# tirr-c/jxl-oxide

Hardware: NVIDIA H100
Metric: Megapixels/s decoded (8K VarDCT d1.0) (higher is better)
Workload: dtype f32

## Files before the change

### jxl_oxide_b200/csrc/kernels/hf_lanes.cuh

```cuda
#pragma once
#include "kernels.h"
#include "stream_common.cuh"
#ifndef __CUDACC__
#include <cstring>
#include <vector>

#include "../launch_tables.h"
#endif

#ifndef JXLB_LANE_TRIP
#define JXLB_LANE_TRIP(is_coefficient)
#endif
#ifndef JXLB_LANE_LZ77_COPIED
#define JXLB_LANE_LZ77_COPIED(n)
#endif

namespace jxlb {
namespace {

#define JXLB_TABLE_QUAL __device__ __constant__ const
namespace hftab {
#include "../host/jxl_tables.inc"
}
#undef JXLB_TABLE_QUAL

__device__ __constant__ const uint8_t kTInfo[27][5] = {
    {1, 1, 0, 0, 1},  {1, 1, 1, 1, 0},  {1, 1, 2, 1, 0},   {1, 1, 3, 1, 0},    {2, 2, 4, 2, 1},   {4, 4, 5, 3, 1},
    {1, 2, 6, 4, 1},  {2, 1, 6, 4, 0},  {1, 4, 7, 5, 1},   {4, 1, 7, 5, 0},    {2, 4, 8, 6, 1},   {4, 2, 8, 6, 0},
    {1, 1, 9, 1, 0},  {1, 1, 9, 1, 0},  {1, 1, 10, 1, 0},  {1, 1, 10, 1, 0},   {1, 1, 10, 1, 0},  {1, 1, 10, 1, 0},
    {8, 8, 11, 7, 1}, {4, 8, 12, 8, 1}, {8, 4, 12, 8, 0},  {16, 16, 13, 9, 1}, {8, 16, 14, 10, 1}, {16, 8, 14, 10, 0},
    {32, 32, 15, 11, 1}, {16, 32, 16, 12, 1}, {32, 16, 16, 12, 0},
};

#ifdef __CUDACC__
struct HfLds {
  using Addr = uint32_t;
  static __device__ __forceinline__ Addr addr(const void* p) { return uint32_t(__cvta_generic_to_shared(p)); }
  static __device__ __forceinline__ uint32_t u8(Addr a) {
    uint32_t v;
    asm("ld.shared.u8 %0, [%1];" : "=r"(v) : "r"(a));
    return v;
  }
  static __device__ __forceinline__ uint32_t u32(Addr a) {
    uint32_t v;
    asm("ld.shared.u32 %0, [%1];" : "=r"(v) : "r"(a));
    return v;
  }
  static __device__ __forceinline__ uint2 u64(Addr a) {
    uint2 v;
    asm("ld.shared.v2.u32 {%0, %1}, [%2];" : "=r"(v.x), "=r"(v.y) : "r"(a));
    return v;
  }
  static __device__ __forceinline__ void st8(Addr a, uint32_t v) { asm volatile("st.shared.u8 [%0], %1;" ::"r"(a), "r"(v)); }
};
#endif

struct HfBits {
  const uint32_t* base;
  uint32_t widx, stop_idx;
  uint64_t buf;
  uint32_t ahead;
  int nbits;
  __device__ __forceinline__ void init(const uint8_t* d, uint64_t bit_pos, uint64_t bit_limit) {
    base = reinterpret_cast<const uint32_t*>(d);
    const uint32_t w = uint32_t(bit_pos >> 5), skip = uint32_t(bit_pos & 31);
    stop_idx = uint32_t((bit_limit + 31) >> 5) + 2;
    buf = uint64_t(__ldg(base + w)) >> skip;
    nbits = 32 - int(skip);
    buf |= uint64_t(__ldg(base + w + 1)) << nbits;
    nbits += 32;
    ahead = __ldg(base + w + 2);
    widx = w + 3;
  }
  __device__ __forceinline__ void refill() {
    buf |= uint64_t(ahead) << nbits;
    nbits += 32;
    ahead = widx <= stop_idx ? __ldg(base + widx) : 0u;
    ++widx;
  }
  __device__ __forceinline__ void top_up() {
    if (nbits < 32) refill();
  }
  __device__ __forceinline__ uint32_t take(uint32_t n) {
    const uint32_t v = uint32_t(buf) & (n >= 32 ? 0xffffffffu : ((1u << n) - 1));
    buf >>= n;
    nbits -= int(n);
    return v;
  }
  __device__ __forceinline__ uint64_t pos() const { return uint64_t(widx - 1) * 32 - uint64_t(nbits); }
  __device__ __forceinline__ bool past_word(uint32_t k) const { return widx > k + (uint32_t(nbits) >> 5); }
};

template <class Mem>
struct HfTables {
  typename Mem::Addr cfg, ans;
  const uint64_t* ans_g;
  const uint32_t* prefix;
  const uint32_t* prefix_meta;
  uint32_t log_alphabet_size, log_bucket, use_prefix;
};

template <class Mem, bool ANS_SMEM, bool PREFIX = true, bool TRACK = false>
__device__ __forceinline__ uint32_t hf_read_value(const HfTables<Mem>& T, HfBits& br, uint32_t& ans_state, uint32_t cl,
                                                  uint32_t past_k = 0, bool* past = nullptr) {
  const uint32_t cfg = Mem::u32(T.cfg + cl * 4);
  uint32_t token;
  if (PREFIX && T.use_prefix) {
    const uint32_t off = __ldg(T.prefix_meta + cl * 2), root_bits = __ldg(T.prefix_meta + cl * 2 + 1);
    const uint32_t peeked = uint32_t(br.buf) & 0x7fffu;
    uint32_t e = __ldg(T.prefix + off + (peeked & ((1u << root_bits) - 1)));
    if (e & 0x80000000u) {
      const uint32_t sb = (e >> 16) & 0xff;
      e = __ldg(T.prefix + off + (1u << root_bits) + (e & 0xffff) + ((peeked >> root_bits) & ((1u << sb) - 1)));
    }
    br.take((e >> 16) & 0xff);
    token = e & 0xffff;
  } else {
    const uint32_t state = ans_state;
    const uint32_t idx = state & 0xfff;
    const uint32_t i = idx >> T.log_bucket;
    const uint32_t pos = idx & ((1u << T.log_bucket) - 1);
    uint2 b;
    if (ANS_SMEM) {
      b = Mem::u64(T.ans + (((cl << T.log_alphabet_size) + i) << 3));
    } else {
      const uint64_t g = __ldg(T.ans_g + ((size_t(cl) << T.log_alphabet_size) + i));
      b = make_uint2(uint32_t(g), uint32_t(g >> 32));
    }
    const bool map_to_alias = pos >= ((b.x >> 8) & 0xff);
    const uint32_t hi = map_to_alias ? b.y : 0u;
    const uint32_t offset = (hi & 0xffff) + pos;
    const uint32_t dist = (b.x >> 16) ^ (hi >> 16);
    token = map_to_alias ? (b.x & 0xff) : i;
    uint32_t next = (state >> 12) * dist + offset;
    if (next < (1u << 16)) {
      if (TRACK) *past |= br.past_word(past_k);
      next = (next << 16) | br.take(16);
    }
    ans_state = next;
  }
  const uint32_t split_exponent = cfg & 0xff;
  const uint32_t split = 1u << split_exponent;
  if (token < split) return token;
  const uint32_t msb = (cfg >> 8) & 0xff, lsb = (cfg >> 16) & 0xff;
  const uint32_t in_token = msb + lsb;
  const uint32_t n = (split_exponent - in_token + ((token - split) >> in_token)) & 31;
  if (TRACK) *past |= br.past_word(past_k);
  br.top_up();
  const uint32_t rest = br.take(n);
  const uint32_t low = token & ((1u << lsb) - 1);
  uint32_t t = (token >> lsb) & ((1u << msb) - 1);
  t |= 1u << msb;
  return uint32_t((((uint64_t(t) << n) | rest) << lsb) | low);
}

struct HfLaneSmem {
  uint32_t ctxlut, small, configs, bctx, cmap, cmap_stride, nz, ans, total;
};
__host__ __device__ inline HfLaneSmem hf_lane_layout(const DevHfParams& p, uint32_t nthreads) {
  HfLaneSmem L;
  uint32_t off = 0;
  auto take = [&](uint32_t bytes) {
    uint32_t o = off;
    off += (bytes + 15) & ~15u;
    return o;
  };
  L.ctxlut = take(128);
  L.small = take((27 + 39) * 4);
  L.configs = take(p.code.num_clusters * 4);
  L.bctx = take(p.block_ctx_map_size);
  L.cmap_stride = 495 * p.num_block_clusters;
  const uint32_t cmap_bytes = L.cmap_stride * p.num_hf_presets;
  L.cmap = cmap_bytes <= kLaneCmapSmemBytes ? take(cmap_bytes) : 0xffffffffu;
  L.nz = take(96 * nthreads);
  uint32_t ab = p.code.use_prefix ? 0 : (p.code.num_clusters << p.code.log_alphabet_size) * 8;
  L.ans = (!p.code.use_prefix && ab <= kHfAnsSmemBytes) ? take(ab) : 0xffffffffu;
  L.total = off;
  return L;
}
__host__ __device__ inline bool hf_lane_staged(const DevHfParams& p, const HfLaneSmem& L) {
  return !p.code.lz77_enabled && !p.code.use_prefix && L.ans != 0xffffffffu && L.cmap != 0xffffffffu;
}

template <class Mem>
struct HfLaneView {
  using Addr = typename Mem::Addr;
  Addr tinfo;
  Addr order_offset;
  Addr ctx;
  Addr bctx;
  Addr nz;
  uint32_t nz_stride;
  Addr cmap;
  HfTables<Mem> code;
  const uint8_t* cmap_ptr;
  CodeView cv;
  uint32_t cmap_stride;
};

__device__ __forceinline__ uint32_t hf_umin(uint32_t a, uint32_t b) { return a < b ? a : b; }
__device__ __forceinline__ uint32_t hf_pack_tinfo(uint32_t t) {
  const uint32_t blocks_log = 31u - uint32_t(__clz(int(uint32_t(kTInfo[t][0]) * kTInfo[t][1])));
  return uint32_t(kTInfo[t][0]) | blocks_log << 8 | uint32_t(kTInfo[t][3]) << 16 | uint32_t(kTInfo[t][4]) << 24;
}
struct HfTinfo {
  uint32_t w8, num_blocks_log, order_id, transpose;
};
__device__ __forceinline__ HfTinfo hf_unpack_tinfo(uint32_t ti) {
  return HfTinfo{ti & 0xff, (ti >> 8) & 0xff, (ti >> 16) & 0xff, ti >> 24};
}

constexpr uint32_t kHfNoBlock = 0xffffffffu;
template <bool SUB>
__device__ __forceinline__ uint32_t hf_block_ctx_cell(const DevFrame& f, const DevHfParams& p, uint32_t bx, uint32_t by) {
  const size_t gi = size_t(by) * f.bw + bx;
  const int32_t t = f.blk_type[gi];
  if (t < 0) return kHfNoBlock;
  const int32_t qf = f.blk_mul[gi];
  const int32_t* thr = p.lf_thresholds;
  uint32_t lf_idx = 0;
  if (p.has_lf_quant) {
    const int32_t* thr_base[3] = {thr, thr + p.num_lf_thr[0], thr + p.num_lf_thr[0] + p.num_lf_thr[1]};
    for (int kk = 0; kk < 3; ++kk) {
      const int cc = kk == 0 ? 0 : (kk == 1 ? 2 : 1);
      lf_idx *= p.num_lf_thr[cc] + 1;
      if (p.num_lf_thr[cc]) {
        const int32_t q = SUB ? f.lf_quant[cc][size_t(by >> f.vshift[cc]) * f.bw + (bx >> f.hshift[cc])] : f.lf_quant[cc][gi];
#pragma unroll 1
        for (uint32_t i = 0; i < p.num_lf_thr[cc]; ++i)
          if (q > thr_base[cc][i]) ++lf_idx;
      }
    }
  }
  uint32_t hf_idx = 0;
#pragma unroll 1
  for (uint32_t i = 0; i < p.num_qf_thr; ++i)
    if (qf > int32_t(p.qf_thresholds[i])) ++hf_idx;
  const uint32_t lf_idx_mul = (p.num_lf_thr[0] + 1) * (p.num_lf_thr[1] + 1) * (p.num_lf_thr[2] + 1);
  return uint32_t(t) | (hf_idx * lf_idx_mul + lf_idx) << 8;
}

struct HfGroupRect {
  uint32_t bx0, by0, width, height;
};
__device__ __forceinline__ HfGroupRect hf_group_rect(const DevFrame& f, const DevHfParams& p, uint32_t group_idx) {
  const uint32_t gb = p.group_dim_blocks;
  HfGroupRect r;
  r.bx0 = group_idx % p.groups_per_row * gb;
  r.by0 = group_idx / p.groups_per_row * gb;
  r.width = hf_umin(gb, f.bw - r.bx0);
  r.height = hf_umin(gb, f.bh - r.by0);
  return r;
}
__device__ __forceinline__ uint2 hf_block_rec(uint32_t info, uint32_t x, uint32_t y) { return make_uint2(info, x | y << 16); }
template <bool SUB>
__device__ __forceinline__ bool hf_block_record(const DevFrame& f, const DevHfParams& p, const HfGroupRect& r, uint32_t i,
                                                uint2& rec) {
  const uint32_t x = i % r.width, y = i / r.width;
  const uint32_t info = hf_block_ctx_cell<SUB>(f, p, r.bx0 + x, r.by0 + y);
  rec = hf_block_rec(info, x, y);
  return info != kHfNoBlock;
}

template <bool SUB, bool STAGED, bool LZ77, class Mem>
__device__ __forceinline__ void hf_lane_stream(const uint8_t* __restrict__ cs, const DevFrame& f, const DevHfParams& p,
                                               const HfLaneView<Mem>& T, const uint2* __restrict__ list, uint32_t count,
                                               const DevHfJob& job, int first_pass, Lz77State* lz, uint64_t* end_bit,
                                               int* status) {
  static_assert(!(LZ77 && STAGED), "LZ77 codes run the general variant");
  using Addr = typename Mem::Addr;
  DevBitReader br;
  HfBits hb;
  int err = kDevOk;
  uint32_t hfp_bits = 0;
  while ((1u << hfp_bits) < p.num_hf_presets) ++hfp_bits;
  uint32_t hfp, ans_state;
  const uint32_t last_word = uint32_t((job.bit_limit + 31) >> 5);
  const uint32_t* stop_word = nullptr;
  bool past = false;
  if (STAGED) {
    hb.init(cs, job.bit_pos, job.bit_limit);
    hfp = hb.take(hfp_bits);
    hb.top_up();
    ans_state = hb.take(32);
    past = (job.bit_pos >> 5) > last_word + 1 || job.bit_pos + hfp_bits > uint64_t(last_word + 2) * 32;
  } else {
    br.init(cs, job.bit_pos, job.bit_limit);
    hfp = br.read(hfp_bits);
    ans_state = p.code.use_prefix ? 0x130000u : br.read(32);
    stop_word = br.origin + last_word + 4;
  }
  if (hfp >= p.num_hf_presets) {
    err = kDevInvalid;
    hfp = 0;
  }
  const uint32_t nbc = p.num_block_clusters;
  const Addr a_cmap = T.cmap + T.cmap_stride * hfp;
  const uint8_t* cluster_map = STAGED ? nullptr : T.cmap_ptr + size_t(T.cmap_stride) * hfp;
  const uint32_t lf_idx_mul = (p.num_lf_thr[0] + 1) * (p.num_lf_thr[1] + 1) * (p.num_lf_thr[2] + 1);
  const uint32_t hf_idx_mul = p.num_qf_thr + 1;

  const HfGroupRect r = hf_group_rect(f, p, job.group_idx);
  const uint32_t bx0 = r.bx0, by0 = r.by0;
  for (uint32_t i = 0; i < 96; ++i) Mem::st8(T.nz + i * T.nz_stride, 0);

  uint32_t x = 0, y = 0;
  uint32_t ci = 3;
  uint32_t w8 = 1, num_blocks = 1, num_blocks_log = 0, order_id = 0, transpose = 0, blk_ctx_idx = 0;
  uint32_t left = count;
  uint2 next = count ? __ldg(list) : make_uint2(0, 0);
  ++list;
  bool in_coeffs = false;
  uint32_t k = 0, size = 0, non_zeros = 0, prev_nonzero = 0, nzc_ctx = 0, block_ctx = 0;
  int c = 0;
  uint32_t sx = 0;
  Addr a_blk = a_cmap;
  const uint8_t* cmap = cluster_map;
  const uint32_t* order = p.orders;
  uint32_t* dst_base = f.coeff[0];

  while (err == kDevOk) {
    uint32_t cl;
    if (!in_coeffs) {
      bool found = false;
      while (!found) {
        if (ci >= 3) {
          if (left == 0) break;
          const uint2 rec = next;
          if (--left) next = __ldg(list++);
          x = rec.y & 0xffff;
          y = rec.y >> 16;
          const HfTinfo ti = hf_unpack_tinfo(Mem::u32(T.tinfo + (rec.x & 0xff) * 4));
          w8 = ti.w8;
          num_blocks_log = ti.num_blocks_log;
          num_blocks = 1u << num_blocks_log;
          order_id = ti.order_id;
          transpose = ti.transpose;
          blk_ctx_idx = rec.x >> 8;
          ci = 0;
        }
        const uint32_t slot = ci++;
        c = slot == 0 ? 1 : (slot == 1 ? 0 : 2);
        sx = x;
        uint32_t sy = y, sbx0 = bx0, sby0 = by0;
        if (SUB) {
          const uint32_t hs = f.hshift[c], vs = f.vshift[c];
          sx = x >> hs, sy = y >> vs, sbx0 = bx0 >> hs, sby0 = by0 >> vs;
          if (hs | vs) {
            if ((sx << hs) != x || (sy << vs) != y) continue;
            if (f.blk_type[size_t(by0 + sy) * f.bw + bx0 + sx] < 0) continue;
            if (num_blocks != 1) {
              err = kDevUnsupported;
              break;
            }
          }
        }
        const uint32_t idx = ((slot * 13 + order_id) * hf_idx_mul) * lf_idx_mul + blk_ctx_idx;
        block_ctx = Mem::u8(T.bctx + idx);
        const uint32_t nz_here = Mem::u8(T.nz + (uint32_t(c) * 32 + sx) * T.nz_stride);
        const uint32_t nz_left = sx ? Mem::u8(T.nz + (uint32_t(c) * 32 + sx - 1) * T.nz_stride) : 0;
        uint32_t predicted;
        if (sy == 0) predicted = sx == 0 ? 32 : nz_left;
        else if (sx == 0) predicted = nz_here;
        else predicted = (nz_here + nz_left + 1) >> 1;
        const uint32_t pidx = predicted >= 8 ? 4 + predicted / 2 : predicted;
        cl = STAGED ? Mem::u8(a_cmap + block_ctx + pidx * nbc) : cluster_map[block_ctx + pidx * nbc];
        dst_base = f.coeff[c] + (size_t(sby0 + sy) * 8) * f.cw + size_t(sbx0 + sx) * 8;
        found = true;
      }
      if (!found) break;
    } else {
      const uint32_t cctx = (nzc_ctx + Mem::u8(T.ctx + ((k - num_blocks) >> num_blocks_log))) * 2 + prev_nonzero;
      if (cctx >= 458) {
        err = kDevInvalid;
        break;
      }
      cl = STAGED ? Mem::u8(a_blk + cctx) : cmap[cctx];
    }

    JXLB_LANE_TRIP(in_coeffs);
    uint32_t value;
    if (STAGED) {
      hb.top_up();
      value = hf_read_value<Mem, true, false, true>(T.code, hb, ans_state, cl, last_word + 3, &past);
    } else {
      if constexpr (LZ77) {
        value = lz77_read_value(T.cv, p.code, *lz, ans_state, br, cl, 0, err);
        if (err != kDevOk) break;
      } else {
        value = cv_read_uint(br, Mem::u32(T.code.cfg + cl * 4), cv_read_symbol(T.cv, ans_state, br, cl));
      }
      past = br.next_word > stop_word;
    }
    if (past) {
      err = kDevOverrun;
      break;
    }

    if (!in_coeffs) {
      if (value > (63u << num_blocks_log)) {
        err = kDevInvalid;
        break;
      }
      const uint32_t nz_val = (value + num_blocks - 1) >> num_blocks_log;
      for (uint32_t dx = 0; dx < w8; ++dx) Mem::st8(T.nz + (uint32_t(c) * 32 + sx + dx) * T.nz_stride, nz_val);
      if (value == 0) continue;
      non_zeros = value;
      prev_nonzero = (non_zeros <= num_blocks * 4) ? 1 : 0;
      order = p.orders + Mem::u32(T.order_offset + (order_id * 3 + c) * 4);
      size = num_blocks * 64;
      if (STAGED) a_blk = a_cmap + block_ctx * 458 + 37 * nbc;
      else cmap = cluster_map + block_ctx * 458 + 37 * nbc;
      nzc_ctx = Mem::u8(T.ctx + 64 + ((non_zeros - 1) >> num_blocks_log));
      k = num_blocks;
      in_coeffs = k < size;
    } else {
      bool channel_done = false;
      if (value == 0) {
        prev_nonzero = 0;
      } else {
        const uint32_t o = __ldg(order + k);
        const uint32_t cvv = uint32_t(dev_unpack_signed(value)) << p.coeff_shift;
        uint32_t dx = o & 0xffff, dy = o >> 16;
        if (transpose) {
          const uint32_t tmp = dx;
          dx = dy;
          dy = tmp;
        }
        uint32_t* dst = dst_base + size_t(dy) * f.cw + dx;
        if (first_pass) *dst = cvv;
        else *dst += cvv;
        prev_nonzero = 1;
        if (--non_zeros == 0) channel_done = true;
        else nzc_ctx = Mem::u8(T.ctx + 64 + ((non_zeros - 1) >> num_blocks_log));
      }
      if (!channel_done && ++k >= size) channel_done = true;
      if (channel_done) {
        in_coeffs = false;
        if ((STAGED ? hb.pos() : br.pos()) > job.bit_limit) err = kDevOverrun;
      }
    }
  }
  const uint64_t end = STAGED ? hb.pos() : br.pos();
  if (err == kDevOk && !p.code.use_prefix && ans_state != 0x130000u) err = kDevBadStream;
  if (err == kDevOk && end > job.bit_limit) err = kDevOverrun;
  *end_bit = end;
  *status = err;
}

#ifndef __CUDACC__
struct HfHostMem {
  using Addr = uintptr_t;
  static Addr addr(const void* p) { return reinterpret_cast<uintptr_t>(p); }
  static uint32_t u8(Addr a) { return *reinterpret_cast<const uint8_t*>(a); }
  static uint32_t u32(Addr a) {
    uint32_t v;
    std::memcpy(&v, reinterpret_cast<const void*>(a), 4);
    return v;
  }
  static uint2 u64(Addr a) {
    uint2 v;
    std::memcpy(&v, reinterpret_cast<const void*>(a), 8);
    return v;
  }
  static void st8(Addr a, uint32_t v) { *reinterpret_cast<uint8_t*>(a) = uint8_t(v); }
};

struct HfLaneTables {
  const uint32_t* tinfo;
  const uint32_t* order_offset;
  const uint8_t* ctx;
  const uint32_t* cfg;
  const uint8_t* bctx;
  const uint8_t* cmap;
  uint32_t cmap_stride;
  CodeView cv;
};

template <bool SUB>
inline void hf_lane_decode(const uint8_t* cs, const DevFrame& f, const DevHfParams& p, const HfLaneTables& T,
                           const uint32_t* blk_ctx, const DevHfJob& job, uint8_t* nz, uint32_t nz_stride, int first_pass,
                           uint64_t* end_bit, int* status) {
  if (p.code.lz77_enabled && f.subsampled) {
    *end_bit = job.bit_pos;
    *status = kDevUnsupported;
    return;
  }
  const HfGroupRect r = hf_group_rect(f, p, job.group_idx);
  std::vector<uint2> list;
  for (uint32_t y = 0; y < r.height; ++y)
    for (uint32_t x = 0; x < r.width; ++x) {
      const uint32_t info = blk_ctx[size_t(r.by0 + y) * f.bw + r.bx0 + x];
      if (info != kHfNoBlock) list.push_back(hf_block_rec(info, x, y));
    }
  HfLaneView<HfHostMem> V;
  V.tinfo = HfHostMem::addr(T.tinfo);
  V.order_offset = HfHostMem::addr(T.order_offset);
  V.ctx = HfHostMem::addr(T.ctx);
  V.bctx = HfHostMem::addr(T.bctx);
  V.nz = HfHostMem::addr(nz);
  V.nz_stride = nz_stride;
  V.cmap = HfHostMem::addr(T.cmap);
  V.cmap_ptr = T.cmap;
  V.cmap_stride = T.cmap_stride;
  V.code.cfg = HfHostMem::addr(T.cfg);
  V.code.ans = HfHostMem::addr(T.cv.ans);
  V.code.ans_g = T.cv.ans;
  V.code.prefix = T.cv.prefix;
  V.code.prefix_meta = T.cv.prefix_meta;
  V.code.log_alphabet_size = T.cv.log_alphabet_size;
  V.code.log_bucket = 12 - T.cv.log_alphabet_size;
  V.code.use_prefix = T.cv.use_prefix;
  V.cv = T.cv;
  const uint2* recs = list.data();
  const uint32_t n = uint32_t(list.size());
  if (p.code.lz77_enabled) {
    std::vector<uint32_t> window(hf_lz77_window_entries(p.group_dim_blocks * 8));
    Lz77State lz;
    lz77_init(lz, window.data(), window.size());
    hf_lane_stream<SUB, false, true>(cs, f, p, V, recs, n, job, first_pass, &lz, end_bit, status);
    JXLB_LANE_LZ77_COPIED(lz.copied);
  } else if (hf_lane_staged(p, hf_lane_layout(p, nz_stride)))
    hf_lane_stream<SUB, true, false>(cs, f, p, V, recs, n, job, first_pass, nullptr, end_bit, status);
  else
    hf_lane_stream<SUB, false, false>(cs, f, p, V, recs, n, job, first_pass, nullptr, end_bit, status);
}
#endif

}
}
```

### jxl_oxide_b200/csrc/kernels/entropy.cu

```cuda
#include "kernels.h"

#include "stream_common.cuh"
#include "hf_lanes.cuh"

namespace jxlb {

namespace {


struct HfSmem {
  uint32_t ctxlut, configs, bctx, cmap, cmap_stride, ans, total;
};
__host__ __device__ inline HfSmem hf_layout(const DevHfParams& p) {
  HfSmem L;
  uint32_t off = 0;
  auto take = [&](uint32_t bytes) {
    uint32_t o = off;
    off += (bytes + 15) & ~15u;
    return o;
  };
  L.ctxlut = take(128);
  L.configs = take(p.code.num_clusters * 4);
  L.bctx = take(p.block_ctx_map_size);
  L.cmap_stride = 495 * p.num_block_clusters;
  L.cmap = take(L.cmap_stride * p.num_hf_presets);
  uint32_t ab = p.code.use_prefix ? 0 : (p.code.num_clusters << p.code.log_alphabet_size) * 8;
  L.ans = (!p.code.use_prefix && ab <= kHfAnsSmemBytes) ? take(ab) : 0xffffffffu;
  L.total = off;
  return L;
}

template <bool SUB, int W, bool ANS_SMEM>
__global__ void __launch_bounds__(W * 32) decode_hf_warp_kernel(const uint8_t* __restrict__ cs, DevFrame f, DevHfParams p,
                                                                const DevHfJob* __restrict__ jobs,
                                                                uint64_t* __restrict__ end_bits, int* __restrict__ status,
                                                                int num_jobs, int first_pass) {
  extern __shared__ __align__(16) uint8_t smem[];
  __shared__ uint32_t s_nz[W][3][32];
  const HfSmem L = hf_layout(p);
  const uint32_t tid = threadIdx.x, nthreads = blockDim.x, lane = tid & 31, warp = tid >> 5;
  uint8_t* s_ctx = smem + L.ctxlut;
  for (uint32_t i = tid; i < 63; i += nthreads) {
    s_ctx[i] = hftab::kCoeffFreqContext[i];
    s_ctx[64 + i] = hftab::kCoeffNumNonzeroContext[i];
  }
  uint32_t* s_cfg = reinterpret_cast<uint32_t*>(smem + L.configs);
  for (uint32_t i = tid; i < p.code.num_clusters; i += nthreads) s_cfg[i] = __ldg(p.code.configs + i);
  uint8_t* s_bctx = smem + L.bctx;
  for (uint32_t i = tid; i < p.block_ctx_map_size; i += nthreads) s_bctx[i] = __ldg(p.block_ctx_map + i);
  {
    uint8_t* dst = smem + L.cmap;
    const uint32_t n = L.cmap_stride * p.num_hf_presets;
    for (uint32_t i = tid; i < n; i += nthreads) dst[i] = __ldg(p.code.cluster_map + i);
  }
  if (ANS_SMEM) {
    uint4* s_ans = reinterpret_cast<uint4*>(smem + L.ans);
    const uint32_t quads = (p.code.num_clusters << p.code.log_alphabet_size) / 2;
    const uint4* src = reinterpret_cast<const uint4*>(p.code.ans);
    for (uint32_t i = tid; i < quads; i += nthreads) s_ans[i] = __ldg(src + i);
  }
  __syncthreads();
  const int job_idx = blockIdx.x * W + int(warp);
  if (job_idx >= num_jobs || lane != 0) return;

  HfTables<HfLds> T;
  T.cfg = HfLds::addr(s_cfg);
  T.ans = ANS_SMEM ? HfLds::addr(smem + L.ans) : 0;
  T.ans_g = p.code.ans;
  T.prefix = p.code.prefix;
  T.prefix_meta = p.code.prefix_meta;
  T.log_alphabet_size = p.code.log_alphabet_size;
  T.log_bucket = 12 - p.code.log_alphabet_size;
  T.use_prefix = p.code.use_prefix;
  const uint32_t a_ctx = HfLds::addr(s_ctx), a_bctx = HfLds::addr(s_bctx);

  const DevHfJob job = jobs[job_idx];
  HfBits br;
  br.init(cs, job.bit_pos, job.bit_limit);
  int err = kDevOk;
  uint32_t hfp_bits = 0;
  while ((1u << hfp_bits) < p.num_hf_presets) ++hfp_bits;
  uint32_t hfp = br.take(hfp_bits);
  if (hfp >= p.num_hf_presets) {
    err = kDevInvalid;
    hfp = 0;
  }
  const uint32_t nbc = p.num_block_clusters;
  const uint32_t a_cmap = HfLds::addr(smem + L.cmap) + hfp * L.cmap_stride;
  const uint32_t lf_idx_mul = (p.num_lf_thr[0] + 1) * (p.num_lf_thr[1] + 1) * (p.num_lf_thr[2] + 1);
  const uint32_t hf_idx_mul = p.num_qf_thr + 1;
  br.top_up();
  uint32_t ans_state = p.code.use_prefix ? 0x130000u : br.take(32);

  const uint32_t gx = job.group_idx % p.groups_per_row, gy = job.group_idx / p.groups_per_row;
  const uint32_t gb = p.group_dim_blocks;
  const uint32_t bx0 = gx * gb, by0 = gy * gb;
  const uint32_t width = min(gb, f.bw - bx0), height = min(gb, f.bh - by0);
  uint32_t(*nz_row)[32] = s_nz[warp];
  for (int c = 0; c < 3; ++c)
    for (int i = 0; i < 32; ++i) nz_row[c][i] = 0;
  const int32_t* thr_base[3] = {p.lf_thresholds, p.lf_thresholds + p.num_lf_thr[0],
                                p.lf_thresholds + p.num_lf_thr[0] + p.num_lf_thr[1]};

  for (uint32_t y = 0; y < height && err == kDevOk; ++y)
    for (uint32_t x = 0; x < width && err == kDevOk; ++x) {
      const size_t gi = size_t(by0 + y) * f.bw + bx0 + x;
      const int32_t t = f.blk_type[gi];
      if (t < 0) continue;
      const int32_t qf = f.blk_mul[gi];
      const uint32_t w8 = kTInfo[t][0], h8 = kTInfo[t][1];
      const uint32_t order_id = kTInfo[t][3];
      const bool transpose = kTInfo[t][4] != 0;
      const uint32_t num_blocks = w8 * h8;
      const uint32_t num_blocks_log = 31u - uint32_t(__clz(int(num_blocks)));
      uint32_t lf_idx = 0;
      if (p.has_lf_quant) {
        const int cs3[3] = {0, 2, 1};
#pragma unroll
        for (int k = 0; k < 3; ++k) {
          const int c = cs3[k];
          lf_idx *= p.num_lf_thr[c] + 1;
          if (p.num_lf_thr[c]) {
            const int32_t q = SUB ? f.lf_quant[c][size_t((by0 + y) >> f.vshift[c]) * f.bw + ((bx0 + x) >> f.hshift[c])] : f.lf_quant[c][gi];
            for (uint32_t i = 0; i < p.num_lf_thr[c]; ++i)
              if (q > thr_base[c][i]) ++lf_idx;
          }
        }
      }
      uint32_t hf_idx = 0;
      for (uint32_t i = 0; i < p.num_qf_thr; ++i)
        if (qf > int32_t(p.qf_thresholds[i])) ++hf_idx;
#pragma unroll 1
      for (int ci = 0; ci < 3 && err == kDevOk; ++ci) {
        const uint32_t ch_idx = uint32_t(ci) * 13 + order_id;
        const int c = (ci == 0) ? 1 : (ci == 1 ? 0 : 2);
        uint32_t sx = x, sy = y, sbx0 = bx0, sby0 = by0;
        if (SUB) {
          const uint32_t hs = f.hshift[c], vs = f.vshift[c];
          sx = x >> hs, sy = y >> vs, sbx0 = bx0 >> hs, sby0 = by0 >> vs;
          if (hs | vs) {
            if ((sx << hs) != x || (sy << vs) != y) continue;
            if (f.blk_type[size_t(by0 + sy) * f.bw + bx0 + sx] < 0) continue;
            if (num_blocks != 1) {
              err = kDevUnsupported;
              break;
            }
          }
        }
        const uint32_t idx = (ch_idx * hf_idx_mul + hf_idx) * lf_idx_mul + lf_idx;
        const uint32_t block_ctx = HfLds::u8(a_bctx + idx);
        uint32_t predicted;
        const uint32_t nz_here = nz_row[c][sx];
        const uint32_t nz_left = sx ? nz_row[c][sx - 1] : 0;
        if (sy == 0) predicted = sx == 0 ? 32 : nz_left;
        else if (sx == 0) predicted = nz_here;
        else predicted = (nz_here + nz_left + 1) >> 1;
        const uint32_t pidx = predicted >= 8 ? 4 + predicted / 2 : predicted;
        br.top_up();
        uint32_t non_zeros = hf_read_value<HfLds, ANS_SMEM>(T, br, ans_state, HfLds::u8(a_cmap + block_ctx + pidx * nbc));
        if (non_zeros > (63u << num_blocks_log)) {
          err = kDevInvalid;
          break;
        }
        const uint32_t nz_val = (non_zeros + num_blocks - 1) >> num_blocks_log;
        for (uint32_t dx = 0; dx < w8; ++dx) nz_row[c][sx + dx] = nz_val;
        if (non_zeros == 0) continue;
        uint32_t prev_nonzero = (non_zeros <= num_blocks * 4) ? 1 : 0;
        const uint32_t* order = p.orders + p.order_offset[order_id * 3 + c];
        const uint32_t size = num_blocks * 64;
        const uint32_t a_blk = a_cmap + block_ctx * 458 + 37 * nbc;
        uint32_t* plane = f.coeff[c];
        const size_t base = (size_t(sby0 + sy) * 8) * f.cw + size_t(sbx0 + sx) * 8;
        uint32_t nzc2 = HfLds::u8(a_ctx + 64 + ((non_zeros - 1) >> num_blocks_log)) * 2;
        for (uint32_t k = num_blocks, i = 0; k < size; ++k, ++i) {
          const uint32_t cctx = nzc2 + HfLds::u8(a_ctx + (i >> num_blocks_log)) * 2 + prev_nonzero;
          if (cctx >= 458) {
            err = kDevInvalid;
            break;
          }
          br.top_up();
          const uint32_t ucoeff = hf_read_value<HfLds, ANS_SMEM>(T, br, ans_state, HfLds::u8(a_blk + cctx));
          if (ucoeff == 0) {
            prev_nonzero = 0;
            continue;
          }
          const uint32_t o = __ldg(order + k);
          const uint32_t cvv = uint32_t(dev_unpack_signed(ucoeff)) << p.coeff_shift;
          uint32_t dx = o & 0xffff, dy = o >> 16;
          if (transpose) {
            const uint32_t tmp = dx;
            dx = dy;
            dy = tmp;
          }
          uint32_t* dst = plane + base + size_t(dy) * f.cw + dx;
          if (first_pass) *dst = cvv;
          else *dst += cvv;
          prev_nonzero = 1;
          if (--non_zeros == 0) break;
          nzc2 = HfLds::u8(a_ctx + 64 + ((non_zeros - 1) >> num_blocks_log)) * 2;
        }
        if (br.pos() > job.bit_limit) err = kDevOverrun;
      }
    }
  if (err == kDevOk && !p.code.use_prefix && ans_state != 0x130000u) err = kDevBadStream;
  if (err == kDevOk && br.pos() > job.bit_limit) err = kDevOverrun;
  end_bits[job_idx] = br.pos();
  status[job_idx] = err;
}


template <bool SUB>
__global__ void __launch_bounds__(256) hf_block_list_kernel(DevFrame f, DevHfParams p, uint2* __restrict__ list,
                                                            uint32_t* __restrict__ counts) {
  __shared__ uint32_t s_warp[8];
  const uint32_t g = blockIdx.x, tid = threadIdx.x, lane = tid & 31, warp = tid >> 5;
  const HfGroupRect r = hf_group_rect(f, p, g);
  const uint32_t n = r.width * r.height;
  uint2* out = list + size_t(g) * p.group_dim_blocks * p.group_dim_blocks;
  uint32_t base = 0;
  for (uint32_t i0 = 0; i0 < n; i0 += 256) {
    uint2 rec;
    const bool has = i0 + tid < n && hf_block_record<SUB>(f, p, r, i0 + tid, rec);
    const uint32_t ballot = __ballot_sync(0xffffffffu, has);
    if (lane == 0) s_warp[warp] = __popc(ballot);
    __syncthreads();
    uint32_t before = base, total = 0;
    for (uint32_t w = 0; w < 8; ++w) {
      before += w < warp ? s_warp[w] : 0;
      total += s_warp[w];
    }
    if (has) out[before + __popc(ballot & ((1u << lane) - 1))] = rec;
    base += total;
    __syncthreads();
  }
  if (tid == 0) counts[g] = base;
}

template <bool SUB, bool STAGED, bool LZ77>
__global__ void __launch_bounds__(128) decode_hf_lanes_kernel(const uint8_t* __restrict__ cs, DevFrame f, DevHfParams p,
                                                              const uint2* __restrict__ list,
                                                              const uint32_t* __restrict__ counts,
                                                              const DevHfJob* __restrict__ jobs,
                                                              uint64_t* __restrict__ end_bits, int* __restrict__ status,
                                                              int num_jobs, int first_pass,
                                                              uint32_t* lz_windows, uint32_t lz_window_len) {
  extern __shared__ __align__(16) uint8_t smem[];
  const uint32_t tid = threadIdx.x, nthreads = blockDim.x;
  const HfLaneSmem L = hf_lane_layout(p, nthreads);
  uint8_t* s_ctx = smem + L.ctxlut;
  for (uint32_t i = tid; i < 63; i += nthreads) {
    s_ctx[i] = hftab::kCoeffFreqContext[i];
    s_ctx[64 + i] = hftab::kCoeffNumNonzeroContext[i];
  }
  uint32_t* s_cfg = reinterpret_cast<uint32_t*>(smem + L.configs);
  for (uint32_t i = tid; i < p.code.num_clusters; i += nthreads) s_cfg[i] = __ldg(p.code.configs + i);
  uint8_t* s_bctx = smem + L.bctx;
  for (uint32_t i = tid; i < p.block_ctx_map_size; i += nthreads) s_bctx[i] = __ldg(p.block_ctx_map + i);
  uint32_t* s_small = reinterpret_cast<uint32_t*>(smem + L.small);
  for (uint32_t i = tid; i < 27; i += nthreads) s_small[i] = hf_pack_tinfo(i);
  for (uint32_t i = tid; i < 39; i += nthreads) s_small[27 + i] = p.order_offset[i];
  HfLaneView<HfLds> T;
  T.tinfo = HfLds::addr(s_small);
  T.order_offset = HfLds::addr(s_small + 27);
  T.ctx = HfLds::addr(s_ctx);
  T.bctx = HfLds::addr(s_bctx);
  T.nz = HfLds::addr(smem + L.nz + tid);
  T.nz_stride = nthreads;
  T.cmap_stride = L.cmap_stride;
  T.cmap = 0;
  T.cmap_ptr = p.code.cluster_map;
  if (L.cmap != 0xffffffffu) {
    uint8_t* s_cmap = smem + L.cmap;
    const uint32_t n = L.cmap_stride * p.num_hf_presets;
    for (uint32_t i = tid; i < n; i += nthreads) s_cmap[i] = __ldg(p.code.cluster_map + i);
    T.cmap = HfLds::addr(s_cmap);
    T.cmap_ptr = s_cmap;
  }
  T.code.cfg = HfLds::addr(s_cfg);
  T.code.ans = 0;
  T.code.ans_g = p.code.ans;
  T.code.prefix = p.code.prefix;
  T.code.prefix_meta = p.code.prefix_meta;
  T.code.log_alphabet_size = p.code.log_alphabet_size;
  T.code.log_bucket = 12 - p.code.log_alphabet_size;
  T.code.use_prefix = p.code.use_prefix;
  T.cv.log_alphabet_size = p.code.log_alphabet_size;
  T.cv.use_prefix = p.code.use_prefix;
  T.cv.configs = s_cfg;
  T.cv.ans = p.code.ans;
  T.cv.prefix = p.code.prefix;
  T.cv.prefix_meta = p.code.prefix_meta;
  if (L.ans != 0xffffffffu) {
    uint4* s_ans = reinterpret_cast<uint4*>(smem + L.ans);
    const uint32_t quads = (p.code.num_clusters << p.code.log_alphabet_size) / 2;
    const uint4* src = reinterpret_cast<const uint4*>(p.code.ans);
    for (uint32_t i = tid; i < quads; i += nthreads) s_ans[i] = __ldg(src + i);
    T.code.ans = HfLds::addr(s_ans);
    T.cv.ans = reinterpret_cast<const uint64_t*>(s_ans);
  }
  __syncthreads();
  const int job_idx = blockIdx.x * int(nthreads) + int(tid);
  if (job_idx >= num_jobs) return;
  const DevHfJob job = jobs[job_idx];
  const uint32_t gb = p.group_dim_blocks;
  if constexpr (LZ77) {
    Lz77State lz;
    lz77_init(lz, lz_windows + size_t(job_idx) * lz_window_len, lz_window_len);
    hf_lane_stream<SUB, STAGED, true>(cs, f, p, T, list + size_t(job.group_idx) * gb * gb, __ldg(counts + job.group_idx),
                                      job, first_pass, &lz, end_bits + job_idx, status + job_idx);
  } else {
    hf_lane_stream<SUB, STAGED, false>(cs, f, p, T, list + size_t(job.group_idx) * gb * gb, __ldg(counts + job.group_idx),
                                       job, first_pass, nullptr, end_bits + job_idx, status + job_idx);
  }
}

}

size_t hf_block_list_count(DevFrame f, DevHfParams p) {
  const uint32_t gb = p.group_dim_blocks;
  return size_t((f.bh + gb - 1) / gb) * p.groups_per_row;
}

void launch_hf_block_list(DevFrame f, DevHfParams p, uint2* list, uint32_t* counts, cudaStream_t stream) {
  const uint32_t groups = uint32_t(hf_block_list_count(f, p));
  if (f.subsampled) hf_block_list_kernel<true><<<groups, 256, 0, stream>>>(f, p, list, counts);
  else hf_block_list_kernel<false><<<groups, 256, 0, stream>>>(f, p, list, counts);
}

void launch_decode_hf_lanes(const uint8_t* cs, DevFrame f, DevHfParams p, const uint2* list, const uint32_t* counts,
                            const DevHfJob* jobs, uint64_t* end_bits, int* status, int num_jobs, int first_pass,
                            int streams_per_cta, cudaStream_t stream, uint32_t* lz_windows, uint32_t lz_window_len) {
  if (num_jobs <= 0) return;
  static const bool attr_set = [] {
    cudaFuncSetAttribute(decode_hf_lanes_kernel<false, false, false>, cudaFuncAttributeMaxDynamicSharedMemorySize, 200 * 1024);
    cudaFuncSetAttribute(decode_hf_lanes_kernel<true, false, false>, cudaFuncAttributeMaxDynamicSharedMemorySize, 200 * 1024);
    cudaFuncSetAttribute(decode_hf_lanes_kernel<false, true, false>, cudaFuncAttributeMaxDynamicSharedMemorySize, 200 * 1024);
    cudaFuncSetAttribute(decode_hf_lanes_kernel<true, true, false>, cudaFuncAttributeMaxDynamicSharedMemorySize, 200 * 1024);
    cudaFuncSetAttribute(decode_hf_lanes_kernel<false, false, true>, cudaFuncAttributeMaxDynamicSharedMemorySize, 200 * 1024);
    return true;
  }();
  (void)attr_set;
  const int nthreads = streams_per_cta <= 64 ? 64 : 128;
  const HfLaneSmem L = hf_lane_layout(p, uint32_t(nthreads));
  const int ctas = (num_jobs + nthreads - 1) / nthreads;
#define JXLB_HF_LANES(SUB_, STAGED_, LZ77_)                                                                        \
  decode_hf_lanes_kernel<SUB_, STAGED_, LZ77_><<<ctas, nthreads, L.total, stream>>>(                               \
      cs, f, p, list, counts, jobs, end_bits, status, num_jobs, first_pass, lz_windows, lz_window_len)
  if (p.code.lz77_enabled) {
    JXLB_HF_LANES(false, false, true);
  } else if (hf_lane_staged(p, L)) {
    if (f.subsampled) JXLB_HF_LANES(true, true, false);
    else JXLB_HF_LANES(false, true, false);
  } else {
    if (f.subsampled) JXLB_HF_LANES(true, false, false);
    else JXLB_HF_LANES(false, false, false);
  }
#undef JXLB_HF_LANES
}

namespace {
template <int W, bool ANS_SMEM>
void launch_hf_warp(const uint8_t* cs, DevFrame f, DevHfParams p, const DevHfJob* jobs, uint64_t* end_bits, int* status,
                    int num_jobs, int first_pass, cudaStream_t stream) {
  static const bool attr_set = [] {
    cudaFuncSetAttribute(decode_hf_warp_kernel<false, W, ANS_SMEM>, cudaFuncAttributeMaxDynamicSharedMemorySize, 200 * 1024);
    cudaFuncSetAttribute(decode_hf_warp_kernel<true, W, ANS_SMEM>, cudaFuncAttributeMaxDynamicSharedMemorySize, 200 * 1024);
    return true;
  }();
  (void)attr_set;
  const HfSmem L = hf_layout(p);
  const int ctas = (num_jobs + W - 1) / W;
  if (f.subsampled)
    decode_hf_warp_kernel<true, W, ANS_SMEM><<<ctas, W * 32, L.total, stream>>>(cs, f, p, jobs, end_bits, status, num_jobs, first_pass);
  else
    decode_hf_warp_kernel<false, W, ANS_SMEM><<<ctas, W * 32, L.total, stream>>>(cs, f, p, jobs, end_bits, status, num_jobs, first_pass);
}
}

void launch_decode_hf(const uint8_t* cs, DevFrame f, DevHfParams p, const DevHfJob* jobs, uint64_t* end_bits, int* status,
                      int num_jobs, int first_pass, int warps_per_cta, cudaStream_t stream) {
  if (num_jobs <= 0) return;
  const bool ans_smem = hf_layout(p).ans != 0xffffffffu;
#define JXLB_HF(W_)                                                                                          \
  do {                                                                                                       \
    if (ans_smem) launch_hf_warp<W_, true>(cs, f, p, jobs, end_bits, status, num_jobs, first_pass, stream);  \
    else launch_hf_warp<W_, false>(cs, f, p, jobs, end_bits, status, num_jobs, first_pass, stream);          \
  } while (0)
  if (warps_per_cta == 32) JXLB_HF(32);
  else if (warps_per_cta == 16) JXLB_HF(16);
  else JXLB_HF(8);
#undef JXLB_HF
}

}
```

Baseline: 8336.

## Speculatively precompute next HF symbol contexts and slot setup ahead of decode

Restructures the per-lane HF coefficient decode loop so the next cluster index is ready before the current symbol is decoded. Both possible next contexts (zero / nonzero) are looked up, along with the next frequency context and order entry. The next block slot (cluster for the nonzero count, destination pointer) is prepared eagerly through a lambda right after each count symbol. This takes the shared-memory lookups off the serial dependency chain between entropy symbols, at the cost of extra speculative loads and register pressure each iteration.

Result: no change. 8376, median of 6 (+0.5%).

```diff
diff --git a/jxl_oxide_b200/csrc/kernels/hf_lanes.cuh b/jxl_oxide_b200/csrc/kernels/hf_lanes.cuh
--- a/jxl_oxide_b200/csrc/kernels/hf_lanes.cuh
+++ b/jxl_oxide_b200/csrc/kernels/hf_lanes.cuh
@@ -10,6 +10,12 @@
 
 #ifndef JXLB_LANE_TRIP
 #define JXLB_LANE_TRIP(is_coefficient)
+#endif
+#ifndef JXLB_LANE_TRIP_BEGIN
+#define JXLB_LANE_TRIP_BEGIN()
+#endif
+#ifndef JXLB_LANE_REGION
+#define JXLB_LANE_REGION(region)
 #endif
 #ifndef JXLB_LANE_LZ77_COPIED
 #define JXLB_LANE_LZ77_COPIED(n)
@@ -54,6 +60,8 @@
   static __device__ __forceinline__ void st8(Addr a, uint32_t v) { asm volatile("st.shared.u8 [%0], %1;" ::"r"(a), "r"(v)); }
 };
 #endif
+
+enum HfLaneRegion { kLaneWalk = 0, kLaneCountTail = 1, kLaneCoeffTail = 2, kLaneCoeffStore = 3 };
 
 struct HfBits {
   const uint32_t* base;
@@ -306,77 +314,92 @@
 
   uint32_t x = 0, y = 0;
   uint32_t ci = 3;
-  uint32_t w8 = 1, num_blocks = 1, num_blocks_log = 0, order_id = 0, transpose = 0, blk_ctx_idx = 0;
+  uint32_t w8 = 1, num_blocks_log = 0, order_id = 0, transpose = 0, blk_ctx_idx = 0;
   uint32_t left = count;
   uint2 next = count ? __ldg(list) : make_uint2(0, 0);
   ++list;
+  int c = 0;
+  uint32_t sx = 0, block_ctx = 0, cl_count = 0;
+  uint32_t* slot_dst = f.coeff[0];
+  bool slot_ready = false;
+  int slot_err = kDevOk;
+  auto prepare_slot = [&]() {
+    JXLB_LANE_REGION(kLaneWalk);
+    slot_ready = false;
+    while (true) {
+      if (ci >= 3) {
+        if (left == 0) return;
+        const uint2 rec = next;
+        if (--left) next = __ldg(list++);
+        x = rec.y & 0xffff;
+        y = rec.y >> 16;
+        const HfTinfo ti = hf_unpack_tinfo(Mem::u32(T.tinfo + (rec.x & 0xff) * 4));
+        w8 = ti.w8;
+        num_blocks_log = ti.num_blocks_log;
+        order_id = ti.order_id;
+        transpose = ti.transpose;
+        blk_ctx_idx = rec.x >> 8;
+        ci = 0;
+      }
+      const uint32_t slot = ci++;
+      c = slot == 0 ? 1 : (slot == 1 ? 0 : 2);
+      sx = x;
+      uint32_t sy = y, sbx0 = bx0, sby0 = by0;
+      if (SUB) {
+        const uint32_t hs = f.hshift[c], vs = f.vshift[c];
+        sx = x >> hs, sy = y >> vs, sbx0 = bx0 >> hs, sby0 = by0 >> vs;
+        if (hs | vs) {
+          if ((sx << hs) != x || (sy << vs) != y) continue;
+          if (f.blk_type[size_t(by0 + sy) * f.bw + bx0 + sx] < 0) continue;
+          if (num_blocks_log != 0) {
+            slot_err = kDevUnsupported;
+            return;
+          }
+        }
+      }
+      const uint32_t idx = ((slot * 13 + order_id) * hf_idx_mul) * lf_idx_mul + blk_ctx_idx;
+      block_ctx = Mem::u8(T.bctx + idx);
+      const uint32_t nz_here = Mem::u8(T.nz + (uint32_t(c) * 32 + sx) * T.nz_stride);
+      const uint32_t nz_left = sx ? Mem::u8(T.nz + (uint32_t(c) * 32 + sx - 1) * T.nz_stride) : 0;
+      uint32_t predicted;
+      if (sy == 0) predicted = sx == 0 ? 32 : nz_left;
+      else if (sx == 0) predicted = nz_here;
+      else predicted = (nz_here + nz_left + 1) >> 1;
+      const uint32_t pidx = predicted >= 8 ? 4 + predicted / 2 : predicted;
+      cl_count = STAGED ? Mem::u8(a_cmap + block_ctx + pidx * nbc) : cluster_map[block_ctx + pidx * nbc];
+      slot_dst = f.coeff[c] + (size_t(sby0 + sy) * 8) * f.cw + size_t(sbx0 + sx) * 8;
+      slot_ready = true;
+      return;
+    }
+  };
+  prepare_slot();
+
   bool in_coeffs = false;
-  uint32_t k = 0, size = 0, non_zeros = 0, prev_nonzero = 0, nzc_ctx = 0, block_ctx = 0;
-  int c = 0;
-  uint32_t sx = 0;
+  uint32_t k = 1, size = 64, non_zeros = 0, nzc_ctx = 0, coef_nbl = 0, coef_nb = 1, coef_transpose = 0;
+  uint32_t cl_coeff = 0;
+  bool bad_ctx = false;
+  uint32_t freq_next = 0;
+  uint32_t o = 0;
   Addr a_blk = a_cmap;
   const uint8_t* cmap = cluster_map;
   const uint32_t* order = p.orders;
   uint32_t* dst_base = f.coeff[0];
 
   while (err == kDevOk) {
-    uint32_t cl;
-    if (!in_coeffs) {
-      bool found = false;
-      while (!found) {
-        if (ci >= 3) {
-          if (left == 0) break;
-          const uint2 rec = next;
-          if (--left) next = __ldg(list++);
-          x = rec.y & 0xffff;
-          y = rec.y >> 16;
-          const HfTinfo ti = hf_unpack_tinfo(Mem::u32(T.tinfo + (rec.x & 0xff) * 4));
-          w8 = ti.w8;
-          num_blocks_log = ti.num_blocks_log;
-          num_blocks = 1u << num_blocks_log;
-          order_id = ti.order_id;
-          transpose = ti.transpose;
-          blk_ctx_idx = rec.x >> 8;
-          ci = 0;
-        }
-        const uint32_t slot = ci++;
-        c = slot == 0 ? 1 : (slot == 1 ? 0 : 2);
-        sx = x;
-        uint32_t sy = y, sbx0 = bx0, sby0 = by0;
-        if (SUB) {
-          const uint32_t hs = f.hshift[c], vs = f.vshift[c];
-          sx = x >> hs, sy = y >> vs, sbx0 = bx0 >> hs, sby0 = by0 >> vs;
-          if (hs | vs) {
-            if ((sx << hs) != x || (sy << vs) != y) continue;
-            if (f.blk_type[size_t(by0 + sy) * f.bw + bx0 + sx] < 0) continue;
-            if (num_blocks != 1) {
-              err = kDevUnsupported;
-              break;
-            }
-          }
-        }
-        const uint32_t idx = ((slot * 13 + order_id) * hf_idx_mul) * lf_idx_mul + blk_ctx_idx;
-        block_ctx = Mem::u8(T.bctx + idx);
-        const uint32_t nz_here = Mem::u8(T.nz + (uint32_t(c) * 32 + sx) * T.nz_stride);
-        const uint32_t nz_left = sx ? Mem::u8(T.nz + (uint32_t(c) * 32 + sx - 1) * T.nz_stride) : 0;
-        uint32_t predicted;
-        if (sy == 0) predicted = sx == 0 ? 32 : nz_left;
-        else if (sx == 0) predicted = nz_here;
-        else predicted = (nz_here + nz_left + 1) >> 1;
-        const uint32_t pidx = predicted >= 8 ? 4 + predicted / 2 : predicted;
-        cl = STAGED ? Mem::u8(a_cmap + block_ctx + pidx * nbc) : cluster_map[block_ctx + pidx * nbc];
-        dst_base = f.coeff[c] + (size_t(sby0 + sy) * 8) * f.cw + size_t(sbx0 + sx) * 8;
-        found = true;
-      }
-      if (!found) break;
-    } else {
-      const uint32_t cctx = (nzc_ctx + Mem::u8(T.ctx + ((k - num_blocks) >> num_blocks_log))) * 2 + prev_nonzero;
-      if (cctx >= 458) {
-        err = kDevInvalid;
-        break;
-      }
-      cl = STAGED ? Mem::u8(a_blk + cctx) : cmap[cctx];
-    }
+    JXLB_LANE_TRIP_BEGIN();
+    if (in_coeffs ? bad_ctx : !slot_ready) {
+      if (in_coeffs) err = kDevInvalid;
+      else err = slot_err;
+      break;
+    }
+    const uint32_t cl = in_coeffs ? cl_coeff : cl_count;
+
+    const uint32_t nzc_less = Mem::u8(T.ctx + 64 + ((non_zeros > 1 ? non_zeros - 2 : 0) >> coef_nbl));
+    const uint32_t cctx0 = (nzc_ctx + freq_next) * 2, cctx1 = (nzc_less + freq_next) * 2 + 1;
+    const uint32_t cl0 = STAGED ? Mem::u8(a_blk + hf_umin(cctx0, 457)) : cmap[hf_umin(cctx0, 457)];
+    const uint32_t cl1 = STAGED ? Mem::u8(a_blk + hf_umin(cctx1, 457)) : cmap[hf_umin(cctx1, 457)];
+    const uint32_t freq_after = Mem::u8(T.ctx + ((k + 2 - coef_nb) >> coef_nbl));
+    const uint32_t o_next = __ldg(order + hf_umin(k + 1, size - 1));
 
     JXLB_LANE_TRIP(in_coeffs);
     uint32_t value;
@@ -398,31 +421,42 @@
     }
 
     if (!in_coeffs) {
+      JXLB_LANE_REGION(kLaneCountTail);
       if (value > (63u << num_blocks_log)) {
         err = kDevInvalid;
         break;
       }
+      const uint32_t num_blocks = 1u << num_blocks_log;
       const uint32_t nz_val = (value + num_blocks - 1) >> num_blocks_log;
       for (uint32_t dx = 0; dx < w8; ++dx) Mem::st8(T.nz + (uint32_t(c) * 32 + sx + dx) * T.nz_stride, nz_val);
-      if (value == 0) continue;
-      non_zeros = value;
-      prev_nonzero = (non_zeros <= num_blocks * 4) ? 1 : 0;
-      order = p.orders + Mem::u32(T.order_offset + (order_id * 3 + c) * 4);
-      size = num_blocks * 64;
-      if (STAGED) a_blk = a_cmap + block_ctx * 458 + 37 * nbc;
-      else cmap = cluster_map + block_ctx * 458 + 37 * nbc;
-      nzc_ctx = Mem::u8(T.ctx + 64 + ((non_zeros - 1) >> num_blocks_log));
-      k = num_blocks;
-      in_coeffs = k < size;
+      if (value != 0) {
+        non_zeros = value;
+        coef_nbl = num_blocks_log;
+        coef_nb = num_blocks;
+        coef_transpose = transpose;
+        order = p.orders + Mem::u32(T.order_offset + (order_id * 3 + c) * 4);
+        size = num_blocks * 64;
+        dst_base = slot_dst;
+        if (STAGED) a_blk = a_cmap + block_ctx * 458 + 37 * nbc;
+        else cmap = cluster_map + block_ctx * 458 + 37 * nbc;
+        nzc_ctx = Mem::u8(T.ctx + 64 + ((non_zeros - 1) >> num_blocks_log));
+        const uint32_t cctx = (nzc_ctx + Mem::u8(T.ctx)) * 2 + (non_zeros <= num_blocks * 4 ? 1 : 0);
+        bad_ctx = cctx >= 458;
+        cl_coeff = STAGED ? Mem::u8(a_blk + hf_umin(cctx, 457)) : cmap[hf_umin(cctx, 457)];
+        freq_next = Mem::u8(T.ctx + (1u >> num_blocks_log));
+        k = num_blocks;
+        o = __ldg(order + k);
+        in_coeffs = true;
+      }
+      prepare_slot();
     } else {
+      JXLB_LANE_REGION(kLaneCoeffTail);
       bool channel_done = false;
-      if (value == 0) {
-        prev_nonzero = 0;
-      } else {
-        const uint32_t o = __ldg(order + k);
+      if (value != 0) {
+        JXLB_LANE_REGION(kLaneCoeffStore);
         const uint32_t cvv = uint32_t(dev_unpack_signed(value)) << p.coeff_shift;
         uint32_t dx = o & 0xffff, dy = o >> 16;
-        if (transpose) {
+        if (coef_transpose) {
           const uint32_t tmp = dx;
           dx = dy;
           dy = tmp;
@@ -430,10 +464,13 @@
         uint32_t* dst = dst_base + size_t(dy) * f.cw + dx;
         if (first_pass) *dst = cvv;
         else *dst += cvv;
-        prev_nonzero = 1;
         if (--non_zeros == 0) channel_done = true;
-        else nzc_ctx = Mem::u8(T.ctx + 64 + ((non_zeros - 1) >> num_blocks_log));
-      }
+        nzc_ctx = nzc_less;
+      }
+      cl_coeff = value != 0 ? cl1 : cl0;
+      bad_ctx = (value != 0 ? cctx1 : cctx0) >= 458;
+      freq_next = freq_after;
+      o = o_next;
       if (!channel_done && ++k >= size) channel_done = true;
       if (channel_done) {
         in_coeffs = false;
```

## Software-pipeline HF coefficient decode: defer stores, prefetch context lookups

Applied to the files above, without the earlier changes.

In the staged HF lane decoder, coefficient stores are deferred by one iteration so the global write overlaps the next symbol read. The next coefficient's frequency context and nonzero-count context are loaded ahead of time. The three per-channel block-context bytes are packed into one register when a block starts. A clock64-based trip probe, compiled only under a define, is added for timing sections. This adds register pressure, and the deferred store must be flushed on every exit path.

Result: no change. 8417 before, 8495 after, median of 6 (+0.9%).

```diff
diff --git a/jxl_oxide_b200/csrc/kernels/entropy.cu b/jxl_oxide_b200/csrc/kernels/entropy.cu
--- a/jxl_oxide_b200/csrc/kernels/entropy.cu
+++ b/jxl_oxide_b200/csrc/kernels/entropy.cu
@@ -392,4 +392,13 @@
 #undef JXLB_HF
 }
 
-}
+#ifdef JXLB_HF_TRIP_PROBE
+extern "C" int jxlb_hf_trip_probe(unsigned long long* out) {
+  unsigned long long zero[kProbeWords] = {};
+  if (cudaDeviceSynchronize() != cudaSuccess) return -1;
+  if (cudaMemcpyFromSymbol(out, g_hf_trip_probe, sizeof(zero)) != cudaSuccess) return -1;
+  return cudaMemcpyToSymbol(g_hf_trip_probe, zero, sizeof(zero)) == cudaSuccess ? int(kProbeWords) : -1;
+}
+#endif
+
+}
diff --git a/jxl_oxide_b200/csrc/kernels/hf_lanes.cuh b/jxl_oxide_b200/csrc/kernels/hf_lanes.cuh
--- a/jxl_oxide_b200/csrc/kernels/hf_lanes.cuh
+++ b/jxl_oxide_b200/csrc/kernels/hf_lanes.cuh
@@ -261,6 +261,75 @@
   rec = hf_block_rec(info, x, y);
   return info != kHfNoBlock;
 }
+
+struct HfPendingCoeff {
+  uint32_t* base;
+  uint32_t order;
+  uint32_t value;
+  bool transpose, pending;
+  __device__ __forceinline__ void store(size_t cw, int first_pass) {
+    uint32_t dx = order & 0xffff, dy = order >> 16;
+    if (transpose) {
+      const uint32_t tmp = dx;
+      dx = dy;
+      dy = tmp;
+    }
+    uint32_t* dst = base + size_t(dy) * cw + dx;
+    if (first_pass) *dst = value;
+    else *dst += value;
+    pending = false;
+  }
+};
+
+#if defined(JXLB_HF_TRIP_PROBE) && defined(__CUDACC__)
+enum {
+  kProbePreCount, kProbePreCoef, kProbeRead, kProbePostCount, kProbePostCoef, kProbeTail, kProbeTrips, kProbeCountTrips,
+  kProbeWords
+};
+__device__ unsigned long long g_hf_trip_probe[kProbeWords];
+struct HfTripProbe {
+  unsigned long long acc[kProbeWords];
+  long long t;
+  bool lead, count;
+  __device__ __forceinline__ void begin() {
+#pragma unroll
+    for (int i = 0; i < kProbeWords; ++i) acc[i] = 0;
+    t = clock64();
+    lead = count = false;
+  }
+  __device__ __forceinline__ void trip(bool on_count) {
+    const long long now = clock64();
+    if (lead) acc[kProbeTail] += now - t;
+    t = now;
+    const uint32_t m = __activemask();
+    lead = (m & ((1u << (threadIdx.x & 31)) - 1)) == 0;
+    count = __any_sync(m, on_count);
+    if (lead) {
+      ++acc[kProbeTrips];
+      if (count) ++acc[kProbeCountTrips];
+    }
+  }
+  template <int SECTION>
+  __device__ __forceinline__ void stamp() {
+    const long long now = clock64();
+    const unsigned long long d = now - t;
+    t = now;
+    if (!lead) return;
+    if (SECTION == 0) (count ? acc[kProbePreCount] : acc[kProbePreCoef]) += d;
+    else if (SECTION == 1) acc[kProbeRead] += d;
+    else (count ? acc[kProbePostCount] : acc[kProbePostCoef]) += d;
+  }
+  __device__ __forceinline__ void end() {
+    if (lead) acc[kProbeTail] += clock64() - t;
+#pragma unroll
+    for (int i = 0; i < kProbeWords; ++i)
+      if (acc[i]) atomicAdd(&g_hf_trip_probe[i], acc[i]);
+  }
+};
+#define JXLB_HF_PROBE(stmt) probe.stmt
+#else
+#define JXLB_HF_PROBE(stmt)
+#endif
 
 template <bool SUB, bool STAGED, bool LZ77, class Mem>
 __device__ __forceinline__ void hf_lane_stream(const uint8_t* __restrict__ cs, const DevFrame& f, const DevHfParams& p,
@@ -318,8 +387,17 @@
   const uint8_t* cmap = cluster_map;
   const uint32_t* order = p.orders;
   uint32_t* dst_base = f.coeff[0];
+  HfPendingCoeff pend;
+  pend.pending = false;
+  uint32_t freq = 0, freq_next = 0, nzc_next = 0;
+  uint32_t bctx3 = 0;
+#if defined(JXLB_HF_TRIP_PROBE) && defined(__CUDACC__)
+  HfTripProbe probe;
+  probe.begin();
+#endif
 
   while (err == kDevOk) {
+    JXLB_HF_PROBE(trip(!in_coeffs));
     uint32_t cl;
     if (!in_coeffs) {
       bool found = false;
@@ -338,6 +416,10 @@
           transpose = ti.transpose;
           blk_ctx_idx = rec.x >> 8;
           ci = 0;
+          if constexpr (STAGED) {
+            const uint32_t b0 = (order_id * hf_idx_mul) * lf_idx_mul + blk_ctx_idx, step = (13 * hf_idx_mul) * lf_idx_mul;
+            bctx3 = Mem::u8(T.bctx + b0) | Mem::u8(T.bctx + b0 + step) << 8 | Mem::u8(T.bctx + b0 + 2 * step) << 16;
+          }
         }
         const uint32_t slot = ci++;
         c = slot == 0 ? 1 : (slot == 1 ? 0 : 2);
@@ -355,8 +437,12 @@
             }
           }
         }
-        const uint32_t idx = ((slot * 13 + order_id) * hf_idx_mul) * lf_idx_mul + blk_ctx_idx;
-        block_ctx = Mem::u8(T.bctx + idx);
+        if constexpr (STAGED) {
+          block_ctx = (bctx3 >> (slot * 8)) & 0xff;
+        } else {
+          const uint32_t idx = ((slot * 13 + order_id) * hf_idx_mul) * lf_idx_mul + blk_ctx_idx;
+          block_ctx = Mem::u8(T.bctx + idx);
+        }
         const uint32_t nz_here = Mem::u8(T.nz + (uint32_t(c) * 32 + sx) * T.nz_stride);
         const uint32_t nz_left = sx ? Mem::u8(T.nz + (uint32_t(c) * 32 + sx - 1) * T.nz_stride) : 0;
         uint32_t predicted;
@@ -370,7 +456,14 @@
       }
       if (!found) break;
     } else {
-      const uint32_t cctx = (nzc_ctx + Mem::u8(T.ctx + ((k - num_blocks) >> num_blocks_log))) * 2 + prev_nonzero;
+      uint32_t cctx;
+      if constexpr (STAGED) {
+        cctx = (nzc_ctx + freq) * 2 + prev_nonzero;
+        freq_next = Mem::u8(T.ctx + ((hf_umin(k + 1, size - 1) - num_blocks) >> num_blocks_log));
+        nzc_next = Mem::u8(T.ctx + 64 + ((non_zeros > 1 ? non_zeros - 2 : 0) >> num_blocks_log));
+      } else {
+        cctx = (nzc_ctx + Mem::u8(T.ctx + ((k - num_blocks) >> num_blocks_log))) * 2 + prev_nonzero;
+      }
       if (cctx >= 458) {
         err = kDevInvalid;
         break;
@@ -378,6 +471,7 @@
       cl = STAGED ? Mem::u8(a_blk + cctx) : cmap[cctx];
     }
 
+    JXLB_HF_PROBE(stamp<0>());
     JXLB_LANE_TRIP(in_coeffs);
     uint32_t value;
     if (STAGED) {
@@ -396,6 +490,10 @@
       err = kDevOverrun;
       break;
     }
+    JXLB_HF_PROBE(stamp<1>());
+    if constexpr (STAGED) {
+      if (pend.pending) pend.store(f.cw, first_pass);
+    }
 
     if (!in_coeffs) {
       if (value > (63u << num_blocks_log)) {
@@ -404,7 +502,10 @@
       }
       const uint32_t nz_val = (value + num_blocks - 1) >> num_blocks_log;
       for (uint32_t dx = 0; dx < w8; ++dx) Mem::st8(T.nz + (uint32_t(c) * 32 + sx + dx) * T.nz_stride, nz_val);
-      if (value == 0) continue;
+      if (value == 0) {
+        JXLB_HF_PROBE(stamp<2>());
+        continue;
+      }
       non_zeros = value;
       prev_nonzero = (non_zeros <= num_blocks * 4) ? 1 : 0;
       order = p.orders + Mem::u32(T.order_offset + (order_id * 3 + c) * 4);
@@ -412,12 +513,19 @@
       if (STAGED) a_blk = a_cmap + block_ctx * 458 + 37 * nbc;
       else cmap = cluster_map + block_ctx * 458 + 37 * nbc;
       nzc_ctx = Mem::u8(T.ctx + 64 + ((non_zeros - 1) >> num_blocks_log));
+      if constexpr (STAGED) freq = Mem::u8(T.ctx);
       k = num_blocks;
       in_coeffs = k < size;
     } else {
       bool channel_done = false;
       if (value == 0) {
         prev_nonzero = 0;
+      } else if constexpr (STAGED) {
+        pend = HfPendingCoeff{dst_base, __ldg(order + k), uint32_t(dev_unpack_signed(value)) << p.coeff_shift,
+                              transpose != 0, true};
+        prev_nonzero = 1;
+        if (--non_zeros == 0) channel_done = true;
+        else nzc_ctx = nzc_next;
       } else {
         const uint32_t o = __ldg(order + k);
         const uint32_t cvv = uint32_t(dev_unpack_signed(value)) << p.coeff_shift;
@@ -434,12 +542,18 @@
         if (--non_zeros == 0) channel_done = true;
         else nzc_ctx = Mem::u8(T.ctx + 64 + ((non_zeros - 1) >> num_blocks_log));
       }
+      if constexpr (STAGED) freq = freq_next;
       if (!channel_done && ++k >= size) channel_done = true;
       if (channel_done) {
         in_coeffs = false;
         if ((STAGED ? hb.pos() : br.pos()) > job.bit_limit) err = kDevOverrun;
       }
     }
+    JXLB_HF_PROBE(stamp<2>());
+  }
+  JXLB_HF_PROBE(end());
+  if constexpr (STAGED) {
+    if (pend.pending) pend.store(f.cw, first_pass);
   }
   const uint64_t end = STAGED ? hb.pos() : br.pos();
   if (err == kDevOk && !p.code.use_prefix && ans_state != 0x130000u) err = kDevBadStream;
```
